# DSXiangLi/ChineseNER

Measured on AMD Instinct MI355X. Metric: training samples/sec, bert_bilstm_crf (BERT-base + BiLSTM + CRF), msra-shaped, higher is better.
Workload: dtype bf16; 1 GPU; model=bert_bilstm_crf, global_batch=64, seq_len=128, parallelism=dp1

## Files before the change

### chinesener_amd/ops/functional.py

```python
from __future__ import annotations

import math
import os
from typing import Optional, Tuple

import torch
import torch.nn.functional as F

from . import reference as ref
from . import hip_enabled, get_ext


def _pad_last(t: torch.Tensor, target: int) -> torch.Tensor:
    d = t.shape[-1]
    return t if d == target else F.pad(t, (0, target - d))


class _LayerNormFn(torch.autograd.Function):
    @staticmethod
    def forward(ctx, x, weight, bias, eps):
        y, mean, rstd = get_ext().layernorm_fwd(x, weight, bias, eps)
        ctx.save_for_backward(x, weight, mean, rstd)
        return y

    @staticmethod
    def backward(ctx, dy):
        x, weight, mean, rstd = ctx.saved_tensors
        dx, dw, db = get_ext().layernorm_bwd(dy.contiguous(), x, weight, mean, rstd)
        return dx, dw, db, None


def layernorm(x, weight, bias, eps: float = 1e-12):
    if hip_enabled(x):
        shape = x.shape
        y = _LayerNormFn.apply(x.reshape(-1, shape[-1]).contiguous(), weight, bias, eps)
        return y.reshape(shape)
    return ref.layernorm(x, weight, bias, eps)


class _AddLayerNormFn(torch.autograd.Function):
    @staticmethod
    def forward(ctx, x, residual, weight, bias, eps):
        y, s, mean, rstd = get_ext().add_layernorm_fwd(x, residual, weight, bias, eps)
        ctx.save_for_backward(s, weight, mean, rstd)
        return y

    @staticmethod
    def backward(ctx, dy):
        s, weight, mean, rstd = ctx.saved_tensors
        dx, dw, db = get_ext().layernorm_bwd(dy.contiguous(), s, weight, mean, rstd)
        return dx, dx, dw, db, None


_rng_counter = None


def _rng_counter_for(device):
    global _rng_counter
    if _rng_counter is None or _rng_counter.device != device:
        seed = torch.initial_seed() & 0x7FFFFFFF
        _rng_counter = torch.tensor([seed], dtype=torch.int64, device=device)
    return _rng_counter


class _DropoutAddLNFn(torch.autograd.Function):

    @staticmethod
    def forward(ctx, x, res, weight, bias, eps, keep):
        y, s, mask, mean, rstd = get_ext().dropout_add_ln_fwd(
            x, res, weight, bias, eps, keep,
            _rng_counter_for(x.device))
        ctx.save_for_backward(s, weight, mask, mean, rstd)
        ctx.keep = keep
        return y

    @staticmethod
    def backward(ctx, dy):
        s, weight, mask, mean, rstd = ctx.saved_tensors
        dsum, dx, dw, db, _ = get_ext().dropout_add_ln_bwd(
            dy.contiguous(), s, weight, mean, rstd, mask, ctx.keep, False)
        return dx, dsum, dw, db, None, None


def dropout_add_layernorm(x, residual, weight, bias, eps: float = 1e-12,
                          p: float = 0.1, training: bool = True):
    if (training and p > 0 and hip_enabled(x) and x.dtype == torch.bfloat16
            and os.environ.get("CHINESENER_NO_FUSED_DROPOUT") != "1"):
        shape = x.shape
        y = _DropoutAddLNFn.apply(
            x.reshape(-1, shape[-1]).contiguous(),
            residual.to(x.dtype).reshape(-1, shape[-1]).contiguous(),
            weight, bias, eps, 1.0 - p)
        return y.reshape(shape)
    if training and p > 0:
        x = F.dropout(x, p, training)
    return add_layernorm(x, residual, weight, bias, eps)


def add_layernorm(x, residual, weight, bias, eps: float = 1e-12):
    if hip_enabled(x):
        shape = x.shape
        y = _AddLayerNormFn.apply(
            x.reshape(-1, shape[-1]).contiguous(),
            residual.to(x.dtype).reshape(-1, shape[-1]).contiguous(),
            weight, bias, eps)
        return y.reshape(shape)
    return ref.add_layernorm(x, residual, weight, bias, eps)


_GEMM_NT_CHOICE: dict = {}
_GEMM_NT_CALLS: dict = {}
_PICK_MIN_RECUR = 6


def _gemm_nt_mode() -> str:
    return os.environ.get("CHINESENER_GEMM_NT", "auto")


def _gemm_nt_ok(x2, w):
    return (x2.shape[0] % 128 == 0 and w.shape[0] % 128 == 0
            and w.shape[1] % 64 == 0 and x2.dtype == torch.bfloat16
            and w.dtype == torch.bfloat16)


def _tuning_active() -> bool:
    try:
        import torch.cuda.tunable as tun
        return tun.is_enabled() and tun.tuning_is_enabled()
    except Exception:
        return False


def _med_time(fn):
    import time as _time
    fn(); fn()
    torch.cuda.synchronize()
    ts = []
    for _ in range(3):
        t0 = _time.perf_counter()
        for _i in range(8):
            fn()
        torch.cuda.synchronize()
        ts.append((_time.perf_counter() - t0) / 8)
    return sorted(ts)[1]


def _pick2(key, fn_ours, fn_lib) -> bool:
    hit = _GEMM_NT_CHOICE.get(key)
    if hit is not None:
        return hit
    if torch.cuda.is_current_stream_capturing() or _tuning_active():
        return False
    n = _GEMM_NT_CALLS.get(key, 0) + 1
    _GEMM_NT_CALLS[key] = n
    if n < _PICK_MIN_RECUR:
        return False

    t_ours, t_lib = _med_time(fn_ours), _med_time(fn_lib)
    _GEMM_NT_CHOICE[key] = bool(t_ours <= t_lib)
    if os.environ.get("CHINESENER_GEMM_DEBUG") == "1":
        import sys
        print(f"[gemm-dispatch] {key}: ours {t_ours*1e6:.1f}us "
              f"lib {t_lib*1e6:.1f}us -> "
              f"{'ours' if _GEMM_NT_CHOICE[key] else 'lib'}",
              file=sys.stderr, flush=True)
    return _GEMM_NT_CHOICE[key]


def _pick_gemm_nt(x2, w, b) -> bool:
    key = (x2.shape[0], w.shape[0], w.shape[1], b is not None)
    hit = _GEMM_NT_CHOICE.get(key)
    if hit is not None:
        return hit
    if torch.cuda.is_current_stream_capturing() or _tuning_active():
        return False
    n = _GEMM_NT_CALLS.get(key, 0) + 1
    _GEMM_NT_CALLS[key] = n
    if n < _PICK_MIN_RECUR:
        return False
    ext = get_ext()

    t_ours = _med_time(lambda: ext.gemm_nt(x2, w, b, False))
    t_lib = _med_time(lambda: F.linear(x2, w, b))
    _GEMM_NT_CHOICE[key] = bool(t_ours <= t_lib)
    if os.environ.get("CHINESENER_GEMM_DEBUG") == "1":
        import sys
        print(f"[gemm-dispatch] fwd {key}: ours {t_ours*1e6:.1f}us "
              f"lib {t_lib*1e6:.1f}us -> "
              f"{'ours' if _GEMM_NT_CHOICE[key] else 'lib'}",
              file=sys.stderr, flush=True)
    return _GEMM_NT_CHOICE[key]


def _linear_fwd(x, w, b):
    mode = _gemm_nt_mode()
    if mode != "off":
        x2 = x.reshape(-1, x.shape[-1])
        if _gemm_nt_ok(x2, w):
            x2 = x2.contiguous()
            wc = w.contiguous()
            if mode == "force" or _pick_gemm_nt(x2, wc, b):
                y = get_ext().gemm_nt(x2, wc, b, False)
                return y.reshape(*x.shape[:-1], w.shape[0])
    return F.linear(x, w, b)


def _linear_dgrad(dyf, x, w):
    M, N = dyf.shape
    K = x.shape[-1]
    mode = _gemm_nt_mode()
    bf16 = dyf.dtype == torch.bfloat16 and x.dtype == torch.bfloat16

    def dx_ours():
        return get_ext().gemm_nt(dyf, w.t().contiguous(), None, False)

    def dx_lib():
        return dyf @ w.to(dyf.dtype)

    if (mode != "off" and bf16 and M % 128 == 0 and K % 128 == 0
            and N % 64 == 0
            and (mode == "force"
                 or _pick2(("dx", M, N, K), dx_ours, dx_lib))):
        return dx_ours().reshape(x.shape)
    return dx_lib().reshape(x.shape)


def _linear_wgrad(dyf, x, w):
    M, N = dyf.shape
    K = x.shape[-1]
    x2 = x.reshape(-1, K)
    mode = _gemm_nt_mode()
    bf16 = dyf.dtype == torch.bfloat16 and x.dtype == torch.bfloat16

    def dw_ours():
        return get_ext().gemm_nt(dyf.t().contiguous(),
                                 x2.t().contiguous(), None, False)

    def dw_lib():
        return dyf.T @ x2

    if (mode != "off" and bf16 and N % 128 == 0 and K % 128 == 0
            and M % 64 == 0
            and (mode == "force"
                 or _pick2(("dw", M, N, K), dw_ours, dw_lib))):
        return dw_ours().to(w.dtype)
    return dw_lib().to(w.dtype)


class _LinearFn(torch.autograd.Function):

    @staticmethod
    def forward(ctx, x, w, b):
        ctx.save_for_backward(x, w)
        ctx.has_bias = b is not None
        return _linear_fwd(x, w, b)

    @staticmethod
    def backward(ctx, dy):
        x, w = ctx.saved_tensors
        dyf = dy.reshape(-1, w.shape[0]).contiguous()
        dx = _linear_dgrad(dyf, x, w)
        dw = _linear_wgrad(dyf, x, w)
        db = get_ext().colsum(dyf) if ctx.has_bias else None
        return dx, dw, db


def linear(x, weight, bias=None):
    if (hip_enabled(x) and x.dtype == weight.dtype
            and not torch.is_autocast_enabled()):
        return _LinearFn.apply(x, weight,
                               bias.to(x.dtype) if bias is not None else None)
    return F.linear(x, weight, bias)


class _LinearDropoutAddLNFn(torch.autograd.Function):

    @staticmethod
    def forward(ctx, x, w, b, res, ln_w, ln_b, eps, keep):
        a = _linear_fwd(x, w, b)
        y, s, mask, mean, rstd = get_ext().dropout_add_ln_fwd(
            a.reshape(-1, a.shape[-1]).contiguous(), res, ln_w, ln_b, eps,
            keep, _rng_counter_for(x.device))
        ctx.save_for_backward(x, w, s, ln_w, mask, mean, rstd)
        ctx.keep = keep
        ctx.has_bias = b is not None
        return y

    @staticmethod
    def backward(ctx, dy):
        x, w, s, ln_w, mask, mean, rstd = ctx.saved_tensors
        dsum, dx_drop, dw_ln, db_ln, dbias = get_ext().dropout_add_ln_bwd(
            dy.contiguous(), s, ln_w, mean, rstd, mask, ctx.keep,
            ctx.has_bias)
        dx = _linear_dgrad(dx_drop, x, w)
        dw = _linear_wgrad(dx_drop, x, w)
        return dx, dw, dbias, dsum, dw_ln, db_ln, None, None


def linear_dropout_add_layernorm(x, weight, bias, residual, ln_w, ln_b,
                                 eps: float = 1e-12, p: float = 0.1,
                                 training: bool = True):
    if (training and p > 0 and hip_enabled(x) and x.dtype == torch.bfloat16
            and weight.dtype == x.dtype
            and (bias is None or bias.dtype == x.dtype)
            and os.environ.get("CHINESENER_NO_FUSED_DROPOUT") != "1"
            and not torch.is_autocast_enabled()):
        H = weight.shape[0]
        y = _LinearDropoutAddLNFn.apply(
            x, weight, bias,
            residual.to(x.dtype).reshape(-1, H).contiguous(),
            ln_w, ln_b, eps, 1.0 - p)
        return y.reshape(*x.shape[:-1], H)
    return dropout_add_layernorm(linear(x, weight, bias), residual, ln_w,
                                 ln_b, eps, p, training)


class _Embed3Fn(torch.autograd.Function):

    @staticmethod
    def forward(ctx, word_w, pos_w, tok_w, token_ids, segment_ids):
        ctx.save_for_backward(token_ids, segment_ids)
        ctx.shapes = (word_w.shape, pos_w.shape, tok_w.shape)
        return get_ext().embed3_fwd(word_w, pos_w, tok_w,
                                    token_ids.contiguous(),
                                    segment_ids.contiguous())

    @staticmethod
    def backward(ctx, dy):
        token_ids, segment_ids = ctx.saved_tensors
        (vs, ps, ts) = ctx.shapes
        B, L, H = dy.shape
        dyf = dy.reshape(-1, H).float()
        dw = torch.zeros(vs, dtype=torch.float32, device=dy.device)
        dw.index_add_(0, token_ids.reshape(-1), dyf)
        dw[0].zero_()
        dp = torch.zeros(ps, dtype=torch.float32, device=dy.device)
        dp[:L] = dy.float().sum(0)
        dt = torch.zeros(ts, dtype=torch.float32, device=dy.device)
        dt.index_add_(0, segment_ids.reshape(-1), dyf)
        return (dw.to(dy.dtype), dp.to(dy.dtype), dt.to(dy.dtype),
                None, None)


def embed3(word_w, pos_w, tok_w, token_ids, segment_ids):
    if (os.environ.get("CHINESENER_NO_EMBED3") != "1"
            and hip_enabled(word_w) and word_w.dtype == torch.bfloat16
            and word_w.shape[1] % 8 == 0
            and token_ids.shape[1] <= pos_w.shape[0]):
        return _Embed3Fn.apply(word_w, pos_w, tok_w, token_ids, segment_ids)
    pos = torch.arange(token_ids.shape[1], device=token_ids.device)
    return (F.embedding(token_ids, word_w, padding_idx=0) + pos_w[pos]
            + F.embedding(segment_ids, tok_w))


class _BiasGeluFn(torch.autograd.Function):
    @staticmethod
    def forward(ctx, x, bias):
        y = get_ext().bias_gelu_fwd(x, bias)
        ctx.save_for_backward(x, bias)
        return y

    @staticmethod
    def backward(ctx, dy):
        x, bias = ctx.saved_tensors
        dx, dbias = get_ext().bias_gelu_bwd(dy.contiguous(), x, bias)
        return dx, dbias


def bias_gelu(x, bias):
    if bias is not None and hip_enabled(x):
        shape = x.shape
        y = _BiasGeluFn.apply(x.reshape(-1, shape[-1]).contiguous(), bias)
        return y.reshape(shape)
    return ref.bias_gelu(x, bias)


def _attn_path(L: int, D: int, dtype, on_gpu: bool) -> str:
    if not on_gpu or dtype != torch.bfloat16 or D > 64 or L < 1:
        return "torch"
    mode = os.environ.get("CHINESENER_ATTN_TILED", "")
    if mode == "force":
        return "tiled" if L <= 512 else "torch"
    if ((L + 31) // 32) * 32 <= 176:
        return "lds"
    if mode != "off" and L <= 512:
        return "tiled"
    return "torch"


class _AttentionFn(torch.autograd.Function):
    @staticmethod
    def forward(ctx, q, k, v, lens, scale, tiled=False):
        ext = get_ext()
        fwd = ext.attn_tiled_fwd if tiled else ext.attn_fwd
        out, lse = fwd(q, k, v, lens, scale, 1.0, None)
        ctx.save_for_backward(q, k, v, out, lse, lens)
        ctx.scale = scale
        ctx.tiled = tiled
        return out

    @staticmethod
    def backward(ctx, dout):
        q, k, v, out, lse, lens = ctx.saved_tensors
        ext = get_ext()
        bwd = ext.attn_tiled_bwd if ctx.tiled else ext.attn_bwd
        dq, dk, dv = bwd(dout.contiguous(), q, k, v, out, lse, lens,
                         ctx.scale, 1.0, None)
        return dq, dk, dv, None, None, None


def attention(q, k, v, mask: Optional[torch.Tensor] = None,
              scale: Optional[float] = None, lens: Optional[torch.Tensor] = None):
    D = q.shape[-1]
    if scale is None:
        scale = 1.0 / math.sqrt(D)
    path = _attn_path(q.shape[2], D, q.dtype, hip_enabled(q))
    if path != "torch":
        Dp = 32 if D <= 32 else 64
        if lens is None:
            lens = (mask.long().sum(1) if mask is not None
                    else torch.full((q.shape[0],), q.shape[2],
                                    dtype=torch.long, device=q.device))
        out = _AttentionFn.apply(_pad_last(q, Dp).contiguous(),
                                 _pad_last(k, Dp).contiguous(),
                                 _pad_last(v, Dp).contiguous(),
                                 lens.to(torch.int32), float(scale),
                                 path == "tiled")
        return out[..., :D] if Dp != D else out
    return ref.attention(q, k, v, mask, scale)


class _AttentionQkvFn(torch.autograd.Function):

    @staticmethod
    def forward(ctx, qkv, lens, scale, keep, tiled=False):
        seed = None
        if keep < 1.0:
            ctr = _rng_counter_for(qkv.device)
            seed = ctr.clone()
            get_ext().bump_counter(ctr)
        ext = get_ext()
        fwd = ext.attn_tiled_fwd_qkv if tiled else ext.attn_fwd_qkv
        out, lse = fwd(qkv, lens, scale, keep, seed)
        ctx.save_for_backward(qkv, out, lse, lens,
                              seed if seed is not None
                              else torch.zeros(0))
        ctx.scale = scale
        ctx.keep = keep
        ctx.tiled = tiled
        return out

    @staticmethod
    def backward(ctx, dout):
        qkv, out, lse, lens, seed = ctx.saved_tensors
        ext = get_ext()
        bwd = ext.attn_tiled_bwd_qkv if ctx.tiled else ext.attn_bwd_qkv
        (dqkv,) = bwd(dout.contiguous(), qkv, out, lse, lens, ctx.scale,
                      ctx.keep, seed if seed.numel() else None)
        return dqkv, None, None, None, None


def attention_qkv(qkv, mask: Optional[torch.Tensor] = None,
                  lens: Optional[torch.Tensor] = None,
                  scale: Optional[float] = None,
                  p_drop: float = 0.0, training: bool = False):
    B, L, _, H, D = qkv.shape
    if scale is None:
        scale = 1.0 / math.sqrt(D)
    keep = 1.0 - p_drop if (training and p_drop > 0) else 1.0
    if os.environ.get("CHINESENER_NO_ATTN_DROP") == "1":
        keep = 1.0
    path = (_attn_path(L, D, qkv.dtype, hip_enabled(qkv))
            if D in (32, 64) else "torch")
    if path != "torch":
        if lens is None:
            lens = (mask.long().sum(1) if mask is not None
                    else torch.full((B,), L, dtype=torch.long,
                                    device=qkv.device))
        return _AttentionQkvFn.apply(qkv.contiguous(), lens.to(torch.int32),
                                     float(scale), float(keep),
                                     path == "tiled")
    q, k, v = (qkv[:, :, i].transpose(1, 2) for i in range(3))
    if keep < 1.0:
        out = ref.attention(q, k, v, mask, scale, p_drop=p_drop,
                            training=training)
    else:
        out = attention(q, k, v, mask=mask, scale=scale, lens=lens)
    return out.transpose(1, 2)


class _LinearAttentionQkvFn(torch.autograd.Function):

    @staticmethod
    def forward(ctx, x, w, b, lens, n_heads, scale, keep):
        B, L = x.shape[0], x.shape[1]
        qkv = _linear_fwd(x, w, b).reshape(B, L, 3, n_heads, -1).contiguous()
        seed = None
        if keep < 1.0:
            ctr = _rng_counter_for(x.device)
            seed = ctr.clone()
            get_ext().bump_counter(ctr)
        out, lse = get_ext().attn_fwd_qkv(qkv, lens, scale, keep, seed)
        ctx.save_for_backward(x, w, b, qkv, out, lse, lens,
                              seed if seed is not None else torch.zeros(0))
        ctx.scale = scale
        ctx.keep = keep
        return out

    @staticmethod
    def backward(ctx, dout):
        x, w, b, qkv, out, lse, lens, seed = ctx.saved_tensors
        dqkv, dbias = get_ext().attn_bwd_qkv_dbias(
            dout.contiguous(), qkv, out, lse, lens, ctx.scale, ctx.keep,
            seed if seed.numel() else None, b)
        dyf = dqkv.reshape(-1, w.shape[0])
        dx = _linear_dgrad(dyf, x, w)
        dw = _linear_wgrad(dyf, x, w)
        return dx, dw, dbias, None, None, None, None


def linear_attention_qkv(x, weight, bias, n_heads: int,
                         mask: Optional[torch.Tensor] = None,
                         lens: Optional[torch.Tensor] = None,
                         p_drop: float = 0.0, training: bool = False):
    B, L = x.shape[0], x.shape[1]
    D = weight.shape[0] // (3 * n_heads)
    if (bias is not None and hip_enabled(x) and x.dtype == torch.bfloat16
            and weight.dtype == x.dtype and bias.dtype == x.dtype
            and not torch.is_autocast_enabled()
            and D in (32, 64) and weight.shape[0] == 3 * n_heads * D
            and _attn_path(L, D, x.dtype, True) == "lds"):
        keep = 1.0 - p_drop if (training and p_drop > 0) else 1.0
        if os.environ.get("CHINESENER_NO_ATTN_DROP") == "1":
            keep = 1.0
        if lens is None:
            lens = (mask.long().sum(1) if mask is not None
                    else torch.full((B,), L, dtype=torch.long,
                                    device=x.device))
        return _LinearAttentionQkvFn.apply(
            x, weight, bias, lens.to(torch.int32), n_heads,
            1.0 / math.sqrt(D), float(keep))
    qkv = linear(x, weight, bias).reshape(B, L, 3, n_heads, -1)
    return attention_qkv(qkv, mask=mask, lens=lens, p_drop=p_drop,
                         training=training)


class _TenerAttentionFn(torch.autograd.Function):

    @staticmethod
    def forward(ctx, qu, qv, k, v, rel, lens):
        out, lse = get_ext().tener_attn_fwd(qu, qv, k, v, rel, lens)
        ctx.save_for_backward(qu, qv, k, v, rel, out, lse, lens)
        return out

    @staticmethod
    def backward(ctx, dout):
        qu, qv, k, v, rel, out, lse, lens = ctx.saved_tensors
        dqu, dqv, dk, dv = get_ext().tener_attn_bwd(
            dout.contiguous(), qu, qv, k, v, rel, out, lse, lens)
        return dqu, dqv, dk, dv, None, None


def tener_attention(q, k, v, u, vb, rel, mask: Optional[torch.Tensor] = None):
    D = q.shape[-1]
    if (hip_enabled(q) and q.dtype == torch.bfloat16 and D <= 32
            and q.shape[2] <= 160):
        lens = (mask.long().sum(1) if mask is not None
                else torch.full((q.shape[0],), q.shape[2], dtype=torch.long,
                                device=q.device))
        qu = _pad_last(q + u[None, :, None, :].to(q.dtype), 32)
        qv = _pad_last(q + vb[None, :, None, :].to(q.dtype), 32)
        out = _TenerAttentionFn.apply(
            qu.contiguous(), qv.contiguous(),
            _pad_last(k, 32).to(torch.bfloat16).contiguous(),
            _pad_last(v, 32).to(torch.bfloat16).contiguous(),
            _pad_last(rel, 32).to(torch.bfloat16).contiguous(),
            lens.to(torch.int32))
        return out[..., :D] if D != 32 else out
    return ref.tener_attention(q, k, v, u, vb, rel, mask)


class _CrfNllFn(torch.autograd.Function):

    @staticmethod
    def forward(ctx, emissions, tags, lens, transitions):
        ll, demis, dtrans = get_ext().crf_fwd(emissions, tags, lens, transitions)
        ctx.save_for_backward(demis, dtrans)
        return ll

    @staticmethod
    def backward(ctx, dll):
        demis, dtrans = ctx.saved_tensors
        return (demis * dll[:, None, None],
                None, None,
                (dtrans * dll[:, None, None]).sum(0))


def crf_nll(emissions, tags, mask, transitions):
    if hip_enabled(emissions):
        lens = mask.long().sum(1).to(torch.int32)
        return _CrfNllFn.apply(emissions.float().contiguous(),
                               tags.to(torch.int32).contiguous(), lens,
                               transitions.float().contiguous())
    return ref.crf_log_likelihood(emissions, tags, mask, transitions)


def crf_viterbi(emissions, mask, transitions):
    if hip_enabled(emissions):
        lens = mask.long().sum(1).to(torch.int32)
        return get_ext().crf_viterbi(emissions.float().contiguous(), lens,
                                     transitions.float().contiguous()).long()
    with torch.no_grad():
        return ref.crf_decode(emissions, mask, transitions)


class _LstmDirFn(torch.autograd.Function):
    @staticmethod
    def forward(ctx, gates_x, w_hh, lens, reverse, act_relu):
        hs, cs, gates = get_ext().lstm_fwd(gates_x, w_hh, lens, reverse, act_relu)
        ctx.save_for_backward(hs, cs, gates, w_hh, lens)
        ctx.flags = (reverse, act_relu)
        return hs

    @staticmethod
    def backward(ctx, dhs):
        hs, cs, gates, w_hh, lens = ctx.saved_tensors
        reverse, act_relu = ctx.flags
        (dgates_x,) = get_ext().lstm_bwd(dhs.contiguous(), hs, cs, gates,
                                         w_hh, lens, reverse, act_relu)
        B, L, h = hs.shape
        if reverse:
            h_prev = torch.cat([hs[:, 1:], torch.zeros_like(hs[:, :1])], dim=1)
        else:
            h_prev = torch.cat([torch.zeros_like(hs[:, :1]), hs[:, :-1]], dim=1)
        dw_hh = h_prev.reshape(-1, h).T @ dgates_x.reshape(-1, 4 * h)
        return dgates_x, dw_hh.to(w_hh.dtype), None, None, None


def _lstm_dir(x, w_ih, w_hh, b, lens, reverse, activation):
    gates_x = (x @ w_ih.to(x.dtype) + b.to(x.dtype))
    return _LstmDirFn.apply(gates_x.contiguous(),
                            w_hh.to(gates_x.dtype).contiguous(),
                            lens.to(torch.int32), bool(reverse),
                            activation == "relu")


class _BiLstmFn(torch.autograd.Function):

    @staticmethod
    def forward(ctx, gates_x, w_hh_f, w_hh_b, lens, act_relu, cell_clip):
        w_hh_t2 = torch.stack([w_hh_f.t(), w_hh_b.t()]) \
            .to(torch.bfloat16).contiguous()
        hs, cs, gates = get_ext().bilstm_fwd(gates_x, w_hh_t2, lens, act_relu,
                                             cell_clip)
        ctx.save_for_backward(hs, cs, gates, w_hh_f, w_hh_b, lens)
        ctx.relu = act_relu
        ctx.cell_clip = cell_clip
        return hs

    @staticmethod
    def backward(ctx, dhs):
        hs, cs, gates, w_hh_f, w_hh_b, lens = ctx.saved_tensors
        w_hh2 = torch.stack([w_hh_f, w_hh_b]).to(torch.bfloat16).contiguous()
        dgates_x = get_ext().bilstm_bwd(dhs.contiguous(), cs, gates, w_hh2,
                                        lens, ctx.relu, ctx.cell_clip)
        h = hs.shape[-1] // 2
        fw, bw = hs[..., :h], hs[..., h:]
        h_prev_f = torch.cat([torch.zeros_like(fw[:, :1]), fw[:, :-1]], 1)
        h_prev_b = torch.cat([bw[:, 1:], torch.zeros_like(bw[:, :1])], 1)
        dg_f = dgates_x[..., :4 * h]
        dg_b = dgates_x[..., 4 * h:]
        dw_f = h_prev_f.reshape(-1, h).T @ dg_f.reshape(-1, 4 * h)
        dw_b = h_prev_b.reshape(-1, h).T @ dg_b.reshape(-1, 4 * h)
        return (dgates_x, dw_f.to(w_hh_f.dtype), dw_b.to(w_hh_b.dtype),
                None, None, None)


def _pad_gates(w, h, hp):
    if h == hp:
        return w
    shape = list(w.shape[:-1])
    wv = w.reshape(*shape, 4, h)
    return F.pad(wv, (0, hp - h)).reshape(*shape, 4 * hp)


def bilstm(x, w_ih_f, w_hh_f, b_f, w_ih_b, w_hh_b, b_b, lens,
           activation: str = "tanh", state_dropout=None,
           cell_clip: float = 0.0):
    h = w_hh_f.shape[0]
    hp = ((h + 31) // 32) * 32
    if hip_enabled(x) and hp <= 256:
        if hp != h:
            w_ih_f = _pad_gates(w_ih_f, h, hp)
            w_ih_b = _pad_gates(w_ih_b, h, hp)
            b_f = _pad_gates(b_f, h, hp)
            b_b = _pad_gates(b_b, h, hp)
            w_hh_f = _pad_gates(F.pad(w_hh_f, (0, 0, 0, hp - h)), h, hp)
            w_hh_b = _pad_gates(F.pad(w_hh_b, (0, 0, 0, hp - h)), h, hp)
        w_ih2 = torch.cat([w_ih_f, w_ih_b], dim=1).to(x.dtype)
        b2 = torch.cat([b_f, b_b]).to(x.dtype)
        gates_x = (x @ w_ih2 + b2).contiguous()
        hs = _BiLstmFn.apply(gates_x, w_hh_f, w_hh_b,
                             lens.to(torch.int32), activation == "relu",
                             float(cell_clip))
        if hp != h:
            hs = torch.cat([hs[..., :h], hs[..., hp:hp + h]], dim=-1)
        return hs
    if x.is_cuda:
        global _LSTM_FALLBACK_WARNED
        if not _LSTM_FALLBACK_WARNED:
            import logging
            logging.getLogger("chinesener_amd").warning(
                "BiLSTM hidden=%d not kernel-eligible (kernel covers "
                "hidden <= 256 via zero-padding); using torch recurrence", h)
            _LSTM_FALLBACK_WARNED = True
    return ref.bilstm_forward(x, w_ih_f, w_hh_f, b_f, w_ih_b, w_hh_b, b_b,
                              lens, activation, state_dropout, cell_clip)


_LSTM_FALLBACK_WARNED = False


class _SoftLexiconFn(torch.autograd.Function):
    @staticmethod
    def forward(ctx, table, ids, weights):
        out = get_ext().softlexicon_fwd(table, ids, weights)
        ctx.save_for_backward(table, ids, weights)
        return out

    @staticmethod
    def backward(ctx, dout):
        table, ids, weights = ctx.saved_tensors
        dtable, dweights = get_ext().softlexicon_bwd(dout.contiguous(), table,
                                                     ids, weights)
        return dtable, None, dweights


def softlexicon_fuse(table, ids, weights):
    if hip_enabled(table):
        out_dtype = table.dtype
        out = _SoftLexiconFn.apply(table.float().contiguous(),
                                   ids.to(torch.int32).contiguous(),
                                   weights.float().contiguous())
        return out.to(out_dtype)
    return ref.softlexicon_fuse(table, ids, weights)


class _MaskedCeFn(torch.autograd.Function):
    @staticmethod
    def forward(ctx, logits, labels, mask):
        loss, probs, nvalid = get_ext().masked_ce_fwd(logits, labels, mask)
        ctx.save_for_backward(probs, labels, mask, nvalid)
        return loss

    @staticmethod
    def backward(ctx, dloss):
        probs, labels, mask, nvalid = ctx.saved_tensors
        dlogits = get_ext().masked_ce_bwd(dloss, probs, labels, mask, nvalid)
        return dlogits, None, None


def masked_cross_entropy(logits, labels, mask):
    if hip_enabled(logits):
        T = logits.shape[-1]
        return _MaskedCeFn.apply(logits.reshape(-1, T).float().contiguous(),
                                 labels.reshape(-1).to(torch.int32).contiguous(),
                                 mask.reshape(-1).to(torch.int32).contiguous())
    return ref.masked_cross_entropy(logits, labels, mask)


def dice_loss(logits, labels, mask, idx_skip: Tuple[int, ...],
              alpha: float = 0.1, gamma: float = 1.0):
    return ref.dice_loss(logits, labels, mask, idx_skip, alpha, gamma)
```

### csrc/bindings.cpp

```cpp
#include <torch/extension.h>

#include <vector>

std::vector<at::Tensor> layernorm_fwd(const at::Tensor&, const at::Tensor&,
                                      const at::Tensor&, double);
std::vector<at::Tensor> add_layernorm_fwd(const at::Tensor&, const at::Tensor&,
                                          const at::Tensor&, const at::Tensor&,
                                          double);
std::vector<at::Tensor> layernorm_bwd(const at::Tensor&, const at::Tensor&,
                                      const at::Tensor&, const at::Tensor&,
                                      const at::Tensor&);
at::Tensor bias_gelu_fwd(const at::Tensor&, const at::Tensor&);
std::vector<at::Tensor> bias_gelu_bwd(const at::Tensor&, const at::Tensor&,
                                      const at::Tensor&);
std::vector<at::Tensor> masked_ce_fwd(const at::Tensor&, const at::Tensor&,
                                      const at::Tensor&);
at::Tensor masked_ce_bwd(const at::Tensor&, const at::Tensor&,
                         const at::Tensor&, const at::Tensor&,
                         const at::Tensor&);
at::Tensor colsum(const at::Tensor&);
std::vector<at::Tensor> dropout_add_ln_fwd(const at::Tensor&,
                                           const at::Tensor&,
                                           const at::Tensor&,
                                           const at::Tensor&, double, double,
                                           const at::Tensor&);
at::Tensor mask_scale(const at::Tensor&, const at::Tensor&, double);
std::vector<at::Tensor> dropout_add_ln_bwd(const at::Tensor&,
                                           const at::Tensor&,
                                           const at::Tensor&,
                                           const at::Tensor&,
                                           const at::Tensor&,
                                           const at::Tensor&, double, bool);
void bump_counter(const at::Tensor&);
at::Tensor wgrad(const at::Tensor&, const at::Tensor&, long);
at::Tensor wgrad2(const at::Tensor&, const at::Tensor&, long);
at::Tensor gemm_nt(const at::Tensor&, const at::Tensor&,
                   c10::optional<at::Tensor>, bool);
at::Tensor embed3_fwd(const at::Tensor&, const at::Tensor&,
                      const at::Tensor&, const at::Tensor&,
                      const at::Tensor&);
std::vector<at::Tensor> crf_fwd(const at::Tensor&, const at::Tensor&,
                                const at::Tensor&, const at::Tensor&);
at::Tensor crf_viterbi(const at::Tensor&, const at::Tensor&,
                       const at::Tensor&);
std::vector<at::Tensor> crf_wide_fwd(const at::Tensor&, const at::Tensor&,
                                     const at::Tensor&, const at::Tensor&);
at::Tensor crf_wide_viterbi(const at::Tensor&, const at::Tensor&,
                            const at::Tensor&);
at::Tensor softlexicon_fwd(const at::Tensor&, const at::Tensor&,
                           const at::Tensor&);
std::vector<at::Tensor> softlexicon_bwd(const at::Tensor&, const at::Tensor&,
                                        const at::Tensor&, const at::Tensor&);
void multi_tensor_adamw(std::vector<at::Tensor>, std::vector<at::Tensor>,
                        std::vector<at::Tensor>, std::vector<at::Tensor>,
                        std::vector<at::Tensor>, std::vector<double>,
                        std::vector<double>, double, double, double,
                        c10::optional<at::Tensor>);
at::Tensor multi_tensor_sumsq(std::vector<at::Tensor>);
void multi_tensor_scale(std::vector<at::Tensor>, const at::Tensor&);
std::vector<at::Tensor> adamw_build_meta(
    std::vector<at::Tensor>, std::vector<at::Tensor>, std::vector<at::Tensor>,
    std::vector<at::Tensor>, std::vector<at::Tensor>, std::vector<double>,
    std::vector<double>);
void multi_tensor_adamw_run(const at::Tensor&, long, long, bool, double,
                            double, double, c10::optional<at::Tensor>);
std::vector<at::Tensor> norm_build_meta(std::vector<at::Tensor>);
at::Tensor multi_tensor_sumsq_run(const at::Tensor&, long, const at::Tensor&);
void multi_tensor_scale_run(const at::Tensor&, long, const at::Tensor&);
void multi_tensor_adamw_tab_run(const at::Tensor&, long, long, bool,
                                std::vector<at::Tensor>,
                                std::vector<c10::optional<at::Tensor>>, double,
                                double, double, c10::optional<at::Tensor>,
                                c10::optional<at::Tensor>);
long grad_table_slots();
long sumsq_chunk_elems();
at::Tensor sumsq_build_chunks(std::vector<long>, std::vector<long>,
                              const at::Tensor&);
at::Tensor multi_tensor_sumsq_coef_run(const at::Tensor&, std::vector<long>,
                                       std::vector<long>,
                                       std::vector<c10::optional<at::Tensor>>,
                                       double);
std::vector<at::Tensor> attn_fwd(const at::Tensor&, const at::Tensor&,
                                 const at::Tensor&, const at::Tensor&, double,
                                 double, c10::optional<at::Tensor>);
std::vector<at::Tensor> attn_bwd(const at::Tensor&, const at::Tensor&,
                                 const at::Tensor&, const at::Tensor&,
                                 const at::Tensor&, const at::Tensor&,
                                 const at::Tensor&, double, double,
                                 c10::optional<at::Tensor>);
std::vector<at::Tensor> attn_fwd_qkv(const at::Tensor&, const at::Tensor&,
                                     double, double,
                                     c10::optional<at::Tensor>);
std::vector<at::Tensor> attn_bwd_qkv(const at::Tensor&, const at::Tensor&,
                                     const at::Tensor&, const at::Tensor&,
                                     const at::Tensor&, double, double,
                                     c10::optional<at::Tensor>);
std::vector<at::Tensor> attn_bwd_qkv_dbias(
    const at::Tensor&, const at::Tensor&, const at::Tensor&,
    const at::Tensor&, const at::Tensor&, double, double,
    c10::optional<at::Tensor>, const at::Tensor&);
std::vector<at::Tensor> attn_tiled_fwd(const at::Tensor&, const at::Tensor&,
                                       const at::Tensor&, const at::Tensor&,
                                       double, double,
                                       c10::optional<at::Tensor>);
std::vector<at::Tensor> attn_tiled_bwd(const at::Tensor&, const at::Tensor&,
                                       const at::Tensor&, const at::Tensor&,
                                       const at::Tensor&, const at::Tensor&,
                                       const at::Tensor&, double, double,
                                       c10::optional<at::Tensor>);
std::vector<at::Tensor> attn_tiled_fwd_qkv(const at::Tensor&,
                                           const at::Tensor&, double, double,
                                           c10::optional<at::Tensor>);
std::vector<at::Tensor> attn_tiled_bwd_qkv(const at::Tensor&,
                                           const at::Tensor&,
                                           const at::Tensor&,
                                           const at::Tensor&,
                                           const at::Tensor&, double, double,
                                           c10::optional<at::Tensor>);
std::vector<at::Tensor> tener_attn_fwd(const at::Tensor&, const at::Tensor&,
                                       const at::Tensor&, const at::Tensor&,
                                       const at::Tensor&, const at::Tensor&);
std::vector<at::Tensor> tener_attn_bwd(const at::Tensor&, const at::Tensor&,
                                       const at::Tensor&, const at::Tensor&,
                                       const at::Tensor&, const at::Tensor&,
                                       const at::Tensor&, const at::Tensor&,
                                       const at::Tensor&);
at::Tensor mfma_probe(const at::Tensor&, const at::Tensor&);
std::vector<at::Tensor> lstm_fwd(const at::Tensor&, const at::Tensor&,
                                 const at::Tensor&, bool, bool);
std::vector<at::Tensor> lstm_bwd(const at::Tensor&, const at::Tensor&,
                                 const at::Tensor&, const at::Tensor&,
                                 const at::Tensor&, const at::Tensor&, bool,
                                 bool);
std::vector<at::Tensor> bilstm_fwd_l(const at::Tensor&, const at::Tensor&,
                                     const at::Tensor&, bool, double);
at::Tensor bilstm_bwd_l(const at::Tensor&, const at::Tensor&,
                        const at::Tensor&, const at::Tensor&,
                        const at::Tensor&, bool, double);

PYBIND11_MODULE(_hip_ops, m) {
  m.doc() = "chinesener_amd gfx950 HIP kernels";
  m.def("layernorm_fwd", &layernorm_fwd);
  m.def("add_layernorm_fwd", &add_layernorm_fwd);
  m.def("layernorm_bwd", &layernorm_bwd);
  m.def("bias_gelu_fwd", &bias_gelu_fwd);
  m.def("bias_gelu_bwd", &bias_gelu_bwd);
  m.def("masked_ce_fwd", &masked_ce_fwd);
  m.def("masked_ce_bwd", &masked_ce_bwd);
  m.def("colsum", &colsum);
  m.def("dropout_add_ln_fwd", &dropout_add_ln_fwd);
  m.def("mask_scale", &mask_scale);
  m.def("dropout_add_ln_bwd", &dropout_add_ln_bwd);
  m.def("bump_counter", &bump_counter);
  m.def("wgrad", &wgrad);
  m.def("wgrad2", &wgrad2);
  m.def("gemm_nt", &gemm_nt, py::arg("a"), py::arg("b"),
        py::arg("bias") = c10::nullopt, py::arg("fp32_out") = false);
  m.def("embed3_fwd", &embed3_fwd);
  m.def("crf_fwd", &crf_fwd);
  m.def("crf_viterbi", &crf_viterbi);
  m.def("softlexicon_fwd", &softlexicon_fwd);
  m.def("softlexicon_bwd", &softlexicon_bwd);
  m.def("multi_tensor_adamw", &multi_tensor_adamw);
  m.def("multi_tensor_sumsq", &multi_tensor_sumsq);
  m.def("multi_tensor_scale", &multi_tensor_scale);
  m.def("adamw_build_meta", &adamw_build_meta);
  m.def("multi_tensor_adamw_run", &multi_tensor_adamw_run);
  m.def("norm_build_meta", &norm_build_meta);
  m.def("multi_tensor_sumsq_run", &multi_tensor_sumsq_run);
  m.def("multi_tensor_scale_run", &multi_tensor_scale_run);
  m.def("multi_tensor_adamw_tab_run", &multi_tensor_adamw_tab_run);
  m.def("sumsq_build_chunks", &sumsq_build_chunks);
  m.def("multi_tensor_sumsq_coef_run", &multi_tensor_sumsq_coef_run);
  m.def("grad_table_slots", &grad_table_slots);
  m.def("sumsq_chunk_elems", &sumsq_chunk_elems);
  m.def("attn_fwd", &attn_fwd);
  m.def("attn_bwd", &attn_bwd);
  m.def("attn_fwd_qkv", &attn_fwd_qkv);
  m.def("attn_bwd_qkv", &attn_bwd_qkv);
  m.def("attn_bwd_qkv_dbias", &attn_bwd_qkv_dbias);
  m.def("attn_tiled_fwd", &attn_tiled_fwd);
  m.def("attn_tiled_bwd", &attn_tiled_bwd);
  m.def("attn_tiled_fwd_qkv", &attn_tiled_fwd_qkv);
  m.def("attn_tiled_bwd_qkv", &attn_tiled_bwd_qkv);
  m.def("tener_attn_fwd", &tener_attn_fwd);
  m.def("tener_attn_bwd", &tener_attn_bwd);
  m.def("mfma_probe", &mfma_probe);
  m.def("lstm_fwd", &lstm_fwd);
  m.def("lstm_bwd", &lstm_bwd);
  m.def("bilstm_fwd", &bilstm_fwd_l);
  m.def("bilstm_bwd", &bilstm_bwd_l);
}
```

### csrc/gemm_nt.hip

```cpp
#include "common.h"

#define BM 128
#define BN 128
#define BK 64

using bfrag = mfma_bf16x8;
using cfrag = mfma_f32x4;

__device__ __forceinline__ cfrag mfma16(bfrag a, bfrag b, cfrag c) {
  return __builtin_amdgcn_mfma_f32_16x16x32_bf16(a, b, c, 0, 0, 0);
}

__device__ __forceinline__ int swz_chunk(int row, int chunk) {
  return chunk ^ (row & 7);
}

__device__ __forceinline__ void stage_tile(const bf16* __restrict__ g,
                                           long ld, long r0, long k0,
                                           bf16* lds) {
  const int t = threadIdx.x;
#pragma unroll
  for (int i = 0; i < 4; ++i) {
    const int lds_off = (t / WAVE) * 4096 + i * 1024 + (t % WAVE) * 16;
    const int row = lds_off >> 7;
    const int chunk = (lds_off & 127) >> 4;
    const long src = (r0 + row) * ld + k0 +
                     (long)(swz_chunk(row, chunk) << 3);
    __builtin_amdgcn_global_load_lds(
        (const __attribute__((address_space(1))) void*)(g + src),
        (__attribute__((address_space(3))) void*)(lds + (lds_off >> 1)),
        16, 0, 0);
  }
}

__device__ __forceinline__ bfrag frag(const bf16* tile, int r0, int k0) {
  const int l = threadIdx.x & (WAVE - 1);
  const int row = r0 + (l & 15);
  const int chunk = (k0 >> 3) + (l >> 4);
  return *reinterpret_cast<const bfrag*>(
      tile + ((long)row << 6) + (swz_chunk(row, chunk) << 3));
}

template <typename OT, bool HAS_BIAS, typename BT>
__global__ __launch_bounds__(256, 2) void gemm_nt_kernel(
    const bf16* __restrict__ A,
    const bf16* __restrict__ B,
    const BT* __restrict__ bias,
    OT* __restrict__ C,
    long M, long N, long K, int tiles_n) {
  __shared__ bf16 smem[2 * 2 * BM * BK];
  bf16* a_s = smem;
  bf16* b_s = smem + 2 * BM * BK;

  const int nwg = gridDim.x;
  int wg = blockIdx.x;
  {
    const int q = nwg >> 3, r = nwg & 7;
    const int xcd = wg & 7, idx = wg >> 3;
    wg = (xcd < r ? xcd * (q + 1) : r * (q + 1) + (xcd - r) * q) + idx;
  }
  const long m0 = (long)(wg / tiles_n) * BM;
  const long n0 = (long)(wg % tiles_n) * BN;

  const int wid = threadIdx.x / WAVE;
  const int wr = (wid >> 1) * 64, wc = (wid & 1) * 64;
  const int lane = threadIdx.x & (WAVE - 1);

  cfrag acc[4][4];
#pragma unroll
  for (int i = 0; i < 4; ++i)
#pragma unroll
    for (int j = 0; j < 4; ++j) acc[i][j] = cfrag{0.f, 0.f, 0.f, 0.f};

  stage_tile(A, K, m0, 0, a_s);
  stage_tile(B, K, n0, 0, b_s);
  __syncthreads();

  const int nkt = (int)(K / BK);
  int buf = 0;
  for (int kt = 0; kt < nkt; ++kt) {
    if (kt + 1 < nkt) {
      const int nxt = buf ^ 1;
      stage_tile(A, K, m0, (long)(kt + 1) * BK, a_s + nxt * BM * BK);
      stage_tile(B, K, n0, (long)(kt + 1) * BK, b_s + nxt * BM * BK);
    }
    const bf16* at = a_s + buf * BM * BK;
    const bf16* bt = b_s + buf * BM * BK;
#pragma unroll
    for (int kk = 0; kk < BK / 32; ++kk) {
      bfrag af[4], bfr[4];
#pragma unroll
      for (int i = 0; i < 4; ++i) af[i] = frag(at, wr + i * 16, kk * 32);
#pragma unroll
      for (int j = 0; j < 4; ++j) bfr[j] = frag(bt, wc + j * 16, kk * 32);
      __builtin_amdgcn_s_setprio(1);
#pragma unroll
      for (int i = 0; i < 4; ++i)
#pragma unroll
        for (int j = 0; j < 4; ++j)
          acc[i][j] = mfma16(af[i], bfr[j], acc[i][j]);
      __builtin_amdgcn_s_setprio(0);
    }
    __syncthreads();
    buf ^= 1;
  }

#pragma unroll
  for (int i = 0; i < 4; ++i) {
    const long row0 = m0 + wr + i * 16 + ((lane >> 4) << 2);
#pragma unroll
    for (int j = 0; j < 4; ++j) {
      const long col = n0 + wc + j * 16 + (lane & 15);
      const float bv = HAS_BIAS ? to_f32(bias[col]) : 0.f;
#pragma unroll
      for (int r = 0; r < 4; ++r)
        from_f32(acc[i][j][r] + bv, &C[(row0 + r) * N + col]);
    }
  }
}

template <typename OT>
static void launch_gemm_nt(const at::Tensor& a, const at::Tensor& b,
                           const c10::optional<at::Tensor>& bias,
                           at::Tensor& out, long M, long N, long K) {
  dim3 grid((unsigned)((M / BM) * (N / BN)));
  if (bias && bias->scalar_type() == at::kBFloat16)
    hipLaunchKernelGGL((gemm_nt_kernel<OT, true, bf16>), grid, dim3(256), 0,
                       cur_stream(a), (const bf16*)a.data_ptr(),
                       (const bf16*)b.data_ptr(),
                       (const bf16*)bias->data_ptr(), (OT*)out.data_ptr(),
                       M, N, K, (int)(N / BN));
  else if (bias)
    hipLaunchKernelGGL((gemm_nt_kernel<OT, true, float>), grid, dim3(256), 0,
                       cur_stream(a), (const bf16*)a.data_ptr(),
                       (const bf16*)b.data_ptr(), bias->data_ptr<float>(),
                       (OT*)out.data_ptr(), M, N, K, (int)(N / BN));
  else
    hipLaunchKernelGGL((gemm_nt_kernel<OT, false, float>), grid, dim3(256), 0,
                       cur_stream(a), (const bf16*)a.data_ptr(),
                       (const bf16*)b.data_ptr(), (const float*)nullptr,
                       (OT*)out.data_ptr(), M, N, K, (int)(N / BN));
}

at::Tensor gemm_nt(const at::Tensor& a, const at::Tensor& b,
                   c10::optional<at::Tensor> bias, bool fp32_out) {
  CHECK_CUDA_CONTIG(a);
  CHECK_CUDA_CONTIG(b);
  TORCH_CHECK(a.scalar_type() == at::kBFloat16 &&
                  b.scalar_type() == at::kBFloat16,
              "gemm_nt: bf16 operands");
  const long M = a.size(0), K = a.size(1), N = b.size(0);
  TORCH_CHECK(b.size(1) == K, "gemm_nt: K mismatch");
  TORCH_CHECK(M % BM == 0 && N % BN == 0 && K % BK == 0,
              "gemm_nt: needs M%128==0, N%128==0, K%64==0 (got ", M, "x", N,
              "x", K, ")");
  if (bias) {
    TORCH_CHECK(bias->is_cuda() && bias->is_contiguous() &&
                    (bias->scalar_type() == at::kFloat ||
                     bias->scalar_type() == at::kBFloat16) &&
                    bias->numel() == N,
                "gemm_nt: bias must be fp32 or bf16 [N]");
  }
  auto out = at::empty({M, N}, a.options().dtype(
                                   fp32_out ? at::kFloat : at::kBFloat16));
  if (fp32_out)
    launch_gemm_nt<float>(a, b, bias, out, M, N, K);
  else
    launch_gemm_nt<bf16>(a, b, bias, out, M, N, K);
  HIP_CHECK_LAST();
  return out;
}
```

Baseline: 4565 samples/sec.

## Add transposed-read GEMM kernels for linear dgrad/wgrad to skip explicit transposes

Adds gemm_nn and gemm_tn HIP kernels that read K-strided operands straight from global memory into swizzled LDS, then build MFMA fragments with the ds_read_tr16 transpose-read instructions. Linear backward dgrad and wgrad call these kernels directly instead of first materialising transposed copies with .t().contiguous(). The wgrad path also picks an automatic split-K factor, with an fp32 workspace and a finishing reduction kernel. This removes the extra transpose copies and adds K-parallelism for wgrad, at the cost of a workspace allocation and an extra reduction pass when split is above 1. It still runs only where the existing autotune picker prefers it over the library GEMM.

```diff
diff --git a/chinesener_amd/ops/functional.py b/chinesener_amd/ops/functional.py
--- a/chinesener_amd/ops/functional.py
+++ b/chinesener_amd/ops/functional.py
@@ -209,10 +209,11 @@
     M, N = dyf.shape
     K = x.shape[-1]
     mode = _gemm_nt_mode()
-    bf16 = dyf.dtype == torch.bfloat16 and x.dtype == torch.bfloat16
+    bf16 = (dyf.dtype == torch.bfloat16 and x.dtype == torch.bfloat16
+            and w.dtype == torch.bfloat16)
 
     def dx_ours():
-        return get_ext().gemm_nt(dyf, w.t().contiguous(), None, False)
+        return get_ext().gemm_nn(dyf.contiguous(), w.contiguous(), False)
 
     def dx_lib():
         return dyf @ w.to(dyf.dtype)
@@ -233,8 +234,7 @@
     bf16 = dyf.dtype == torch.bfloat16 and x.dtype == torch.bfloat16
 
     def dw_ours():
-        return get_ext().gemm_nt(dyf.t().contiguous(),
-                                 x2.t().contiguous(), None, False)
+        return get_ext().gemm_tn(dyf.contiguous(), x2.contiguous(), 0, False)
 
     def dw_lib():
         return dyf.T @ x2
diff --git a/csrc/bindings.cpp b/csrc/bindings.cpp
--- a/csrc/bindings.cpp
+++ b/csrc/bindings.cpp
@@ -36,6 +36,8 @@
 at::Tensor wgrad2(const at::Tensor&, const at::Tensor&, long);
 at::Tensor gemm_nt(const at::Tensor&, const at::Tensor&,
                    c10::optional<at::Tensor>, bool);
+at::Tensor gemm_tn(const at::Tensor&, const at::Tensor&, long, bool);
+at::Tensor gemm_nn(const at::Tensor&, const at::Tensor&, bool);
 at::Tensor embed3_fwd(const at::Tensor&, const at::Tensor&,
                       const at::Tensor&, const at::Tensor&,
                       const at::Tensor&);
@@ -156,6 +158,10 @@
   m.def("wgrad2", &wgrad2);
   m.def("gemm_nt", &gemm_nt, py::arg("a"), py::arg("b"),
         py::arg("bias") = c10::nullopt, py::arg("fp32_out") = false);
+  m.def("gemm_tn", &gemm_tn, py::arg("a"), py::arg("b"),
+        py::arg("split") = 0, py::arg("fp32_out") = false);
+  m.def("gemm_nn", &gemm_nn, py::arg("a"), py::arg("b"),
+        py::arg("fp32_out") = false);
   m.def("embed3_fwd", &embed3_fwd);
   m.def("crf_fwd", &crf_fwd);
   m.def("crf_viterbi", &crf_viterbi);
diff --git a/csrc/gemm_nt.hip b/csrc/gemm_nt.hip
--- a/csrc/gemm_nt.hip
+++ b/csrc/gemm_nt.hip
@@ -170,3 +170,249 @@
   HIP_CHECK_LAST();
   return out;
 }
+
+__device__ __forceinline__ int swz_ks(int row) {
+  return ((row & 3) << 2) | ((row >> 2) & 3);
+}
+
+__device__ __forceinline__ void stage_tile_ks(const bf16* __restrict__ g,
+                                              long ld, long k0, long c0,
+                                              bf16* lds) {
+  const int t = threadIdx.x;
+#pragma unroll
+  for (int i = 0; i < 4; ++i) {
+    const int lds_off = (t / WAVE) * 4096 + i * 1024 + (t % WAVE) * 16;
+    const int row = lds_off >> 8;
+    const int slot = (lds_off & 255) >> 4;
+    const long src = (k0 + row) * ld + c0 + (long)((slot ^ swz_ks(row)) << 3);
+    __builtin_amdgcn_global_load_lds(
+        (const __attribute__((address_space(1))) void*)(g + src),
+        (__attribute__((address_space(3))) void*)(lds + (lds_off >> 1)),
+        16, 0, 0);
+  }
+}
+
+__device__ __forceinline__ int tr_off(int r0, int c0) {
+  const int l = threadIdx.x & (WAVE - 1);
+  const int row = r0 + ((l & 15) >> 2);
+  const int col = c0 + ((l & 3) << 2);
+  return (row << 7) + (((col >> 3) ^ swz_ks(row)) << 3) + (col & 7);
+}
+
+__device__ __forceinline__ bfrag frag_tr(const bf16* tile, int off_lo,
+                                         int off_hi) {
+  typedef __attribute__((address_space(3))) s16x4 lds_s16x4;
+  const s16x4 lo =
+      __builtin_amdgcn_ds_read_tr16_b64_v4i16((lds_s16x4*)(tile + off_lo));
+  const s16x4 hi =
+      __builtin_amdgcn_ds_read_tr16_b64_v4i16((lds_s16x4*)(tile + off_hi));
+  const s16x8 f = __builtin_shufflevector(lo, hi, 0, 1, 2, 3, 4, 5, 6, 7);
+  return __builtin_bit_cast(bfrag, f);
+}
+
+template <bool A_KMAJOR, typename OT>
+__global__ __launch_bounds__(256, 2) void gemm_ks_kernel(
+    const bf16* __restrict__ A, const bf16* __restrict__ B,
+    OT* __restrict__ C,
+    long M, long N, long K, int tiles_n, int tiles, int split) {
+  __shared__ __attribute__((aligned(16))) bf16 smem[2 * 2 * BM * BK];
+  bf16* a_s = smem;
+  bf16* b_s = smem + 2 * BM * BK;
+
+  const int nwg = gridDim.x;
+  int wg = blockIdx.x;
+  {
+    const int q = nwg >> 3, r = nwg & 7;
+    const int xcd = wg & 7, idx = wg >> 3;
+    wg = (xcd < r ? xcd * (q + 1) : r * (q + 1) + (xcd - r) * q) + idx;
+  }
+  const int s = wg / tiles, tile = wg - s * tiles;
+  const long m0 = (long)(tile / tiles_n) * BM;
+  const long n0 = (long)(tile % tiles_n) * BN;
+
+  const int wid = threadIdx.x / WAVE;
+  const int wr = (wid >> 1) * 64, wc = (wid & 1) * 64;
+  const int lane = threadIdx.x & (WAVE - 1);
+  const int g8 = (lane >> 4) << 3;
+
+  int aoff[4][2], boff[4][2];
+#pragma unroll
+  for (int i = 0; i < 4; ++i) {
+    aoff[i][0] = tr_off(g8, wr + i * 16);
+    aoff[i][1] = tr_off(g8 + 4, wr + i * 16);
+    boff[i][0] = tr_off(g8, wc + i * 16);
+    boff[i][1] = tr_off(g8 + 4, wc + i * 16);
+  }
+
+  cfrag acc[4][4];
+#pragma unroll
+  for (int i = 0; i < 4; ++i)
+#pragma unroll
+    for (int j = 0; j < 4; ++j) acc[i][j] = cfrag{0.f, 0.f, 0.f, 0.f};
+
+  const int nkt = (int)(K / BK);
+  const int kb = (int)((long)s * nkt / split);
+  const int ke = (int)((long)(s + 1) * nkt / split);
+
+  if (A_KMAJOR) stage_tile(A, K, m0, (long)kb * BK, a_s);
+  else stage_tile_ks(A, M, (long)kb * BK, m0, a_s);
+  stage_tile_ks(B, N, (long)kb * BK, n0, b_s);
+  __syncthreads();
+
+  int buf = 0;
+  for (int kt = kb; kt < ke; ++kt) {
+    const bf16* at = a_s + buf * BM * BK;
+    const bf16* bt = b_s + buf * BM * BK;
+    bfrag af[BK / 32][4], bfr[BK / 32][4];
+#pragma unroll
+    for (int kk = 0; kk < BK / 32; ++kk) {
+#pragma unroll
+      for (int i = 0; i < 4; ++i)
+        af[kk][i] = A_KMAJOR ? frag(at, wr + i * 16, kk * 32)
+                             : frag_tr(at + kk * 32 * 128, aoff[i][0],
+                                       aoff[i][1]);
+#pragma unroll
+      for (int j = 0; j < 4; ++j)
+        bfr[kk][j] = frag_tr(bt + kk * 32 * 128, boff[j][0], boff[j][1]);
+    }
+    if (kt + 1 < ke) {
+      const int nxt = buf ^ 1;
+      const long k1 = (long)(kt + 1) * BK;
+      if (A_KMAJOR) stage_tile(A, K, m0, k1, a_s + nxt * BM * BK);
+      else stage_tile_ks(A, M, k1, m0, a_s + nxt * BM * BK);
+      stage_tile_ks(B, N, k1, n0, b_s + nxt * BM * BK);
+    }
+    __builtin_amdgcn_s_setprio(1);
+#pragma unroll
+    for (int kk = 0; kk < BK / 32; ++kk)
+#pragma unroll
+      for (int i = 0; i < 4; ++i)
+#pragma unroll
+        for (int j = 0; j < 4; ++j)
+          acc[i][j] = mfma16(af[kk][i], bfr[kk][j], acc[i][j]);
+    __builtin_amdgcn_s_setprio(0);
+    __syncthreads();
+    buf ^= 1;
+  }
+
+  OT* Cs = C + (long)s * M * N;
+#pragma unroll
+  for (int i = 0; i < 4; ++i) {
+    const long row0 = m0 + wr + i * 16 + ((lane >> 4) << 2);
+#pragma unroll
+    for (int j = 0; j < 4; ++j) {
+      const long col = n0 + wc + j * 16 + (lane & 15);
+#pragma unroll
+      for (int r = 0; r < 4; ++r)
+        from_f32(acc[i][j][r], &Cs[(row0 + r) * N + col]);
+    }
+  }
+}
+
+template <typename OT>
+__global__ __launch_bounds__(256) void splitk_finish_kernel(
+    const float* __restrict__ part, OT* __restrict__ out, long n4,
+    long slab, int split) {
+  const long i = (long)blockIdx.x * blockDim.x + threadIdx.x;
+  if (i >= n4) return;
+  f32x4 acc = reinterpret_cast<const f32x4*>(part)[i];
+  for (int s = 1; s < split; ++s)
+    acc += reinterpret_cast<const f32x4*>(part + (long)s * slab)[i];
+#pragma unroll
+  for (int e = 0; e < 4; ++e) from_f32(acc[e], &out[i * 4 + e]);
+}
+
+static int choose_split(long tiles, long nkt, long MN) {
+  static const int cand[] = {1, 2, 3, 4, 6, 8};
+  int best = 1;
+  double best_cost = 1e30;
+  for (int c : cand) {
+    if (c > nkt) break;
+    const double waves = (double)((tiles * c + 511) / 512);
+    const double stages = (double)((nkt + c - 1) / c);
+    double cost = waves * stages * 0.7;
+    if (tiles * c < 256) cost *= 0.75;
+    if (c > 1) cost += 2.0 + (double)c * MN * 8.0 / 6.0e6;
+    if (cost < best_cost) { best_cost = cost; best = c; }
+  }
+  return best;
+}
+
+template <bool A_KMAJOR>
+static at::Tensor launch_gemm_ks(const at::Tensor& a, const at::Tensor& b,
+                                 long M, long N, long K, int split,
+                                 bool fp32_out) {
+  const int tiles_n = (int)(N / BN), tiles = (int)((M / BM) * tiles_n);
+  auto out = at::empty({M, N}, a.options().dtype(
+                                   fp32_out ? at::kFloat : at::kBFloat16));
+  auto st = cur_stream(a);
+  const bf16* ap = (const bf16*)a.data_ptr();
+  const bf16* bp = (const bf16*)b.data_ptr();
+  if (split == 1) {
+    if (fp32_out)
+      hipLaunchKernelGGL((gemm_ks_kernel<A_KMAJOR, float>), dim3(tiles),
+                         dim3(256), 0, st, ap, bp, out.data_ptr<float>(), M,
+                         N, K, tiles_n, tiles, 1);
+    else
+      hipLaunchKernelGGL((gemm_ks_kernel<A_KMAJOR, bf16>), dim3(tiles),
+                         dim3(256), 0, st, ap, bp, (bf16*)out.data_ptr(), M,
+                         N, K, tiles_n, tiles, 1);
+    HIP_CHECK_LAST();
+    return out;
+  }
+  auto ws = at::empty({(long)split, M, N}, a.options().dtype(at::kFloat));
+  hipLaunchKernelGGL((gemm_ks_kernel<A_KMAJOR, float>),
+                     dim3((unsigned)(tiles * split)), dim3(256), 0, st, ap,
+                     bp, ws.data_ptr<float>(), M, N, K, tiles_n, tiles,
+                     split);
+  HIP_CHECK_LAST();
+  const long n4 = M * N / 4;
+  dim3 fgrid((unsigned)((n4 + 255) / 256));
+  if (fp32_out)
+    hipLaunchKernelGGL((splitk_finish_kernel<float>), fgrid, dim3(256), 0, st,
+                       ws.data_ptr<float>(), out.data_ptr<float>(), n4,
+                       M * N, split);
+  else
+    hipLaunchKernelGGL((splitk_finish_kernel<bf16>), fgrid, dim3(256), 0, st,
+                       ws.data_ptr<float>(), (bf16*)out.data_ptr(), n4,
+                       M * N, split);
+  HIP_CHECK_LAST();
+  return out;
+}
+
+at::Tensor gemm_tn(const at::Tensor& a, const at::Tensor& b, long split,
+                   bool fp32_out) {
+  CHECK_CUDA_CONTIG(a);
+  CHECK_CUDA_CONTIG(b);
+  TORCH_CHECK(a.dim() == 2 && b.dim() == 2 &&
+                  a.scalar_type() == at::kBFloat16 &&
+                  b.scalar_type() == at::kBFloat16,
+              "gemm_tn: 2-D bf16 operands");
+  const long T = a.size(0), M = a.size(1), N = b.size(1);
+  TORCH_CHECK(b.size(0) == T, "gemm_tn: T mismatch");
+  TORCH_CHECK(T > 0 && M > 0 && N > 0 && M % BM == 0 && N % BN == 0 &&
+                  T % BK == 0,
+              "gemm_tn: needs M%128==0, N%128==0, T%64==0 (got ", M, "x", N,
+              "x", T, ")");
+  const long nkt = T / BK;
+  TORCH_CHECK(split >= 0 && split <= 16 && split <= nkt,
+              "gemm_tn: split must be 0 (auto) or 1..min(16, T/64)");
+  if (split == 0) split = choose_split((M / BM) * (N / BN), nkt, M * N);
+  return launch_gemm_ks<false>(a, b, M, N, T, (int)split, fp32_out);
+}
+
+at::Tensor gemm_nn(const at::Tensor& a, const at::Tensor& b, bool fp32_out) {
+  CHECK_CUDA_CONTIG(a);
+  CHECK_CUDA_CONTIG(b);
+  TORCH_CHECK(a.dim() == 2 && b.dim() == 2 &&
+                  a.scalar_type() == at::kBFloat16 &&
+                  b.scalar_type() == at::kBFloat16,
+              "gemm_nn: 2-D bf16 operands");
+  const long M = a.size(0), K = a.size(1), N = b.size(1);
+  TORCH_CHECK(b.size(0) == K, "gemm_nn: K mismatch");
+  TORCH_CHECK(M > 0 && N > 0 && K > 0 && M % BM == 0 && N % BN == 0 &&
+                  K % BK == 0,
+              "gemm_nn: needs M%128==0, N%128==0, K%64==0 (got ", M, "x", N,
+              "x", K, ")");
+  return launch_gemm_ks<true>(a, b, M, N, K, 1, fp32_out);
+}
```

Result: faster. 5112 samples/sec, median of 6 (+12.0%).
